# smly/RiichiEnv

Hardware: AMD Instinct MI355X
Metric: env.step()/s (whole node) at 65 536 parallel 4p games; bit-exact MJAI parity (higher is better)
Workload: dtype u8

## Files before the change

riichienv_amd/csrc/rmj_step4.hip.h:

```cpp
namespace RMJ_NS {

#define R4_LIST 16
#define R4_ACT_CAP (KSANMA ? 2 * R4_LIST : R4_LIST)
#define R4_RE_DRAW 1u
#define R4_RE_RESTART 2u
#define R4_RE_PUB 3u
#define R4_RE_YAKU_CLAIMS 4u
#define R4_RE_YAKU_TSUMO 5u
#define R4_RE_WIN_TSUMO 6u
#define R4_RE_WIN_RON 7u
#define R4_RET_ROUND 0x100u
#define STEP_F_ROWS_SHIFT 20
__device__ __forceinline__ uint32_t r4_rows(uint32_t flags) {
    const uint32_t c = (flags >> STEP_F_ROWS_SHIFT) & 3u;
    return c == 0u ? 4u : c;
}
#ifdef RMJ_CUTS
#define R4M(id) do { if (rmj::g_cut == (id)) asm volatile("s_endpgm" ::: "memory"); } while (0)
#define R4BAIL(q, id) do { (q).bail = true; if ((q).r == 0) atomicAdd(&rmj::g_bail_reason[id], 1u); } while (0)
#else
#define R4M(id) do {} while (0)
#ifdef RMJ_CENSUS
#define R4BAIL(q, id) do { (q).bail = true; (q).why = (id); } while (0)
#elif defined(RMJ_TL4)
// ... 939 lines not shown
            need_tp = false;
        }
        if (RICH && __ballot(need_tp)) {
            if (need_tp) {
                tp = r4_tenpai_keep(q, P, full, hl);
                if (r == 0 && !r_stage) { G->tp_seat = (uint8_t)pid; G->tp_mask = (uint16_t)tp; G->tp_step = G->step_count + 1u; }
            }
        }
        const bool ok = r < hl && !forb && (!r_stage || ((tp >> r) & 1u));
        const uint32_t vb = rballot(ok, rb);
        if (ok) r4_put(q, pid, n + __popc(vb & ((1u << r) - 1u)), mk_action(RMJ_DISCARD, ht, 0), r4_tile_id(hty));
        n += __popc(vb);
        if (riichi_pre && tp != 0u) {
            if (r == 0) r4_put(q, pid, n, mk_action(RMJ_RIICHI, RMJ_TILE_NONE, 0), KSANMA ? 27 : 37);
            n += 1;
        }
    }
    R4M(61);
    if (drawable > 0 && drawn) {
        if (!r_decl && !r_stage) {
            const bool any4 = (((full.a | full.b | full.c) & O9_4) | (full.d & O7_4)) != 0u;
            if (any4) {
                const int next_t = __builtin_amdgcn_update_dpp(0xFFFF, ht, 0x101 , 0xf, 0xf, false);
                if (rballot(r < hl - 2 && ht > next_t, rb)) { R4BAIL(q, 15); return; }
                const int prev_ty = __builtin_amdgcn_update_dpp(-1, hty, 0x111 , 0xf, 0xf, false);
                const bool is4 = r < hl - 1 && hty != prev_ty && ph_cnt(full, hty) == 4;
                const uint32_t ab = rballot(is4, rb);
                if (is4) {
                    const uint32_t lo = (uint32_t)hty * 4u;
                    r4_put(q, pid, n + __popc(ab & ((1u << r) - 1u)), mk_action(RMJ_ANKAN, lo, 4, lo, lo + 1, lo + 2, lo + 3),
                           (KSANMA ? 29 : 42) + r4_tile_id(hty));
                }
                n += __popc(ab);
            }
            const uint32_t pon_lane = rballot(r < nmelds && P->meld_type[r & 3] == RMJ_MELD_PON, rb);
            if (pon_lane) {
                for (int m = 0; m < nmelds; m++) {
                    if (P->meld_type[m] != RMJ_MELD_PON) continue;
                    const int target = P->meld_tiles[m][0] >> 2;
                    const bool hit = r < hl && hty == target;
                    const uint32_t kb = rballot(hit, rb);
                    if (hit)
                        r4_put(q, pid, n + __popc(kb & ((1u << r) - 1u)),
                               mk_kakan(ht, P->meld_tiles[m][0], P->meld_tiles[m][1], P->meld_tiles[m][2]),
                               (KSANMA ? 29 : 42) + r4_tile_id(target));
                    n += __popc(kb);
                }
            }
        } else if (r_decl) {
            if (ph_cnt(full, drawn_tile >> 2) == 4) { R4BAIL(q, 16); return; }
        }
    }
    if (G->is_first_turn && !r_stage && (G->p[0].n_melds | G->p[1].n_melds | G->p[2].n_melds | G->p[3].n_melds) == 0) {
        const bool term = r < hl && is_terminal_tile136(ht);
        const uint32_t lo = row_or16(term && hty < 32 ? 1u << hty : 0u), hi = row_or16(term && hty >= 32 ? 1u << (hty - 32) : 0u);
        const int kinds = __popc((uint32_t)rbc((int)lo, rb + 15)) + __popc((uint32_t)rbc((int)hi, rb + 15));
        if (kinds >= 9) {
            if (r == 0) r4_put(q, pid, n, mk_action(RMJ_KYUSHU, RMJ_TILE_NONE, 0), KSANMA ? 57 : 80);
            n += 1;
        }
    }
    if (KSANMA && drawn && drawable > 0) {
        const bool hit = r < hl && hty == 30;
        const uint32_t kb = rballot(hit, rb);
        if (hit) r4_put(q, pid, n + __popc(kb & ((1u << r) - 1u)), mk_action(RMJ_KITA, ht, 0), 59);
        n += __popc(kb);
    }
    if (n > R4_ACT_CAP) { R4BAIL(q, 17); return; }
    nl_mine = r == pid ? n : 0;
    wave_sync();
}

__device__ __forceinline__ void r4_emit_now(R4& q, bool on, uint32_t w) {
    if (q.E->skip_log) return;
    const uint32_t evc = q.G->ev_count;
    wave_sync();
    if (on) {
        uint32_t* dst = reinterpret_cast<uint32_t*>(q.E->events + (size_t)q.g * (q.E->ring_mask + 1u) + (evc & q.E->ring_mask));
        if (q.r < 8) dst[q.r] = q.r == 7 ? ((w & 0x00FFFFFFu) | ((uint32_t)KNP << 24)) : w;
        if (q.r == 0) q.G->ev_count = evc + 1u;
    }
    wave_sync();
}
#ifdef RMJ_RE_PROF
#define RE_MARK(k) do { const unsigned long long t__ = __builtin_amdgcn_s_memrealtime(); if (lane == 0) atomicAdd(&rmj::g_re_prof[k], t__ - re_t); re_t = t__; } while (0)
#define RE_ROWS(md) do { if ((threadIdx.x & 15u) == 0u) atomicAdd(&rmj::g_re_prof[8 + ((md) & 15u)], 1ull); } while (0)
#define RE_STAMP(t) const unsigned long long t = __builtin_amdgcn_s_memrealtime()
#define RE_ROUND_END_DONE(t) do { if ((threadIdx.x & 63u) == 0u) { const unsigned long long tr = __builtin_amdgcn_s_memrealtime(); atomicAdd(&rmj::g_re_prof[0], tr - t); atomicAdd(&rmj::g_re_prof[1], 1ull); atomicAdd(&rmj::g_re_prof[17], t); atomicAdd(&rmj::g_re_prof[19], tr); } } while (0)
#define RE_PASS2_DONE(t) do { if ((threadIdx.x & 63u) == 0u) { atomicAdd(&rmj::g_re_prof[2], __builtin_amdgcn_s_memrealtime() - t); atomicAdd(&rmj::g_re_prof[3], 1ull); } } while (0)
#else
#define RE_MARK(k) do {} while (0)
#define RE_ROWS(md) do {} while (0)
#define RE_STAMP(t) do {} while (0)
#define RE_ROUND_END_DONE(t) do {} while (0)
#define RE_PASS2_DONE(t) do {} while (0)
#endif
template <bool RICH>
__device__ __noinline__ void r4_round_end(const Env* Ep, uint32_t g0) {
    const int lane = threadIdx.x & 63, row = lane >> 4, r = lane & 15, rb = lane & 48;
#ifdef RMJ_RE_PROF
    unsigned long long re_t = __builtin_amdgcn_s_memrealtime();
    if (lane == 0) atomicAdd(&rmj::g_re_prof[16], re_t);
#endif
    Quad4Shared& sh = g_q4;
    const uint32_t mode = sh.rmode[row];
    CEnv& E = *(CEnv*)uni_ptr(Ep);
    g0 = uni(g0);
    GState* G = &sh.st[row];
    R4 q;
    q.G = G; q.T = &sh.u.t; q.E = &E; q.lane = lane; q.r = r; q.rb = rb; q.row = row; q.g = g0 + (uint32_t)row;
    q.live = mode != 0u; q.bail = false; q.cont = 0; q.rend = mode; q.evn = 0; q.dirty = 0xFu; q.pause_ok = false; q.yk = 0u; q.yk_mode = 0u; q.gf = false;
    const bool draw = mode == R4_RE_DRAW, restart = mode == R4_RE_RESTART;
    const bool win_t = mode == R4_RE_WIN_TSUMO, win_r = mode == R4_RE_WIN_RON, win = win_t || win_r;
    bool newround = restart;
    int n_oya = 0, n_rw = 0, n_honba = 0;
    uint32_t n_sticks = 0u;
    const bool seat = r < KNP;
    const int oya = G->oya;
    bool oya_won = false;
    if (RICH && __ballot(win)) {
        const uint8_t* Wg = E.wall + (size_t)q.g * RMJ_WALL_STRIDE;
        const uint32_t rules = E.rule_bits;
        const bool from_discard = G->last_discard_pid != 0xFF;
        const int target = (win_r && from_discard) ? (int)G->last_discard_pid : (int)G->current_player;
        const int win_tile = win_t ? (G->drawn_tile != 0xFF ? (int)G->drawn_tile : 0) : (from_discard ? (int)G->last_discard_tile : 0);
        const uint32_t ron_m = win_r ? (sh.yk[row] & 0xFu) : 0u;
        const uint32_t honba0 = G->honba;
        int32_t total_d = 0;
        bool honba_taken = false, deposit_taken = false;
        for (int dist = 0; dist < KNP; dist++) {
            int w = target + dist;
            w = w >= KNP ? w - KNP : w;
            const bool on = dist == 0 ? win_t : (win_r && ((ron_m >> w) & 1u) != 0u);
            if (!__ballot(on)) continue;
            const PState& Wp = G->p[w & 3];
            const uint32_t wfl = on ? (uint32_t)Wp.flags : 0u;
            const bool riichi = (wfl & PF_RIICHI_DECLARED) != 0u;
            uint32_t cf = (riichi ? CF_RIICHI : 0u) | ((wfl & PF_DOUBLE_RIICHI) ? CF_DOUBLE_RIICHI : 0u) | ((wfl & PF_IPPATSU) ? CF_IPPATSU : 0u);
            const bool last_tile = G->drawable_count == 0 && !G->is_rinshan;
            if (win_t) {
                cf |= CF_TSUMO;
                if (last_tile) cf |= CF_HAITEI;
                if (G->is_rinshan) cf |= CF_RINSHAN;
                const bool no_melds = (G->p[0].n_melds | G->p[1].n_melds | G->p[2].n_melds | G->p[3].n_melds) == 0;
                if (G->is_first_turn && no_melds) cf |= CF_FIRST_TURN;
            } else {
                if (last_tile) cf |= CF_HOUTEI;
                if (G->pending_kan_pid != 0xFF && a_type(G->pending_kan_action) != RMJ_KITA) cf |= CF_CHANKAN;
            }
            const uint32_t hb = honba_taken ? 0u : honba0;
            if (on) honba_taken = true;
            E4Out o = r4_seat_eval<true>(on ? 1u : 0u, (uint32_t)w, (uint32_t)win_tile, cf, hb, riichi, Wg);
            const bool w_oya = w == oya;
            if (o.yakuman && o.han > 13) {
                int cap = 0;
                if (((o.ym >> 47) & 1ull) && !(rules & RMJ_RULE_JUNSEI_CHUUREN_DOUBLE)) cap += 13;
                if (((o.ym >> 48) & 1ull) && !(rules & RMJ_RULE_SUUANKOU_TANKI_DOUBLE)) cap += 13;
                if (((o.ym >> 49) & 1ull) && !(rules & RMJ_RULE_KOKUSHI13_DOUBLE)) cap += 13;
                if (((o.ym >> 50) & 1ull) && !(rules & RMJ_RULE_DAISUUSHII_DOUBLE)) cap += 13;
                if (cap > 0) {
                    const int hh = o.han > cap ? o.han - cap : 0;
                    o.han = hh < 13 ? 13 : hh;
                    const ScoreOut s2 = calc_score((uint32_t)o.han, 0u, w_oya, win_t, hb, (uint32_t)KNP);
                    o.ron = s2.ron; o.tsumo_oya = s2.tsumo_oya; o.tsumo_ko = s2.tsumo_ko;
                }
            }
            const bool won = on && o.is_win;
            int total_val = 0, pao_val = 0, pao_seat = -1;
            if (won && o.yakuman) {
                const uint64_t ids = (0x7FFull << 35) | (0xFull << 47);
                total_val = __popcll(o.ym & ids);
                if (((o.ym >> 47) & 1ull) && (rules & RMJ_RULE_JUNSEI_CHUUREN_DOUBLE)) total_val += 1;
                if (((o.ym >> 48) & 1ull) && (rules & RMJ_RULE_SUUANKOU_TANKI_DOUBLE)) total_val += 1;
                if (((o.ym >> 49) & 1ull) && (rules & RMJ_RULE_KOKUSHI13_DOUBLE)) total_val += 1;
                const int v50 = (rules & RMJ_RULE_DAISUUSHII_DOUBLE) ? 2 : 1;
                if (((o.ym >> 50) & 1ull) && v50 == 2) total_val += 1;
                if (((o.ym >> 37) & 1ull) && Wp.pao37 != 0xFF) { pao_val += 1; pao_seat = Wp.pao37; }
                if (((o.ym >> 50) & 1ull) && Wp.pao50 != 0xFF) { pao_val += v50; pao_seat = Wp.pao50; }
            }
            const int32_t sticks = (won && !deposit_taken) ? (int32_t)(G->riichi_sticks * 1000u) : 0;
            int32_t d = 0;
// ... 311 lines not shown
        }
        wave_sync();
#pragma unroll
        for (int k = 0; k < 3; k++) {
            const int i = lane + 64 * k;
            if (i < N) {
                const uint32_t b = (uint32_t)(key[k] >> 57);
                const uint32_t kw = (((uint32_t)(key[k] >> 49) & 0xFFu) << 8) | (uint32_t)i;
                const int lo = off8[b], hi = b == 127u ? N : (int)off8[b + 1u];
                int rk = lo;
                for (int t = lo; t < hi; t++) {
                    const uint32_t kt = gk[t];
                    bool less = kt < kw;
                    if ((kt >> 8) == (kw >> 8) && kt != kw) {
                        const uint32_t it = kt & 0xFFu;
                        const uint64_t kf = sm64(hs + (uint64_t)it * 0x9E3779B97F4A7C15ull);
                        less = kf < key[k] || (kf == key[k] && it < (uint32_t)i);
                    }
                    rk += less ? 1 : 0;
                }
                place(rk, (KSANMA && i >= 4) ? i + 28 : i);
            }
        }
        if (lane < (RMJ_WALL_STRIDE - N)) Wg[N + lane] = 0;
        }
        wave_sync();
        {
            const int sp = lane >> 4, sl = lane & 15;
            const bool in = sp < KNP && sl < 13;
            const int t = in ? (int)Gb->p[sp & 3].hand[sl] : 0xFFFF;
            int rk = 0;
#pragma unroll
            for (int k = 0; k < 13; k++) rk += rbc(t, rb + k) < t ? 1 : 0;
            wave_sync();
            if (in) Gb->p[sp & 3].hand[rk] = (uint8_t)t;
            if (sp < KNP && sl == 0) Gb->p[sp & 3].hand_len = sp == oya ? 14 : 13;
        }
        if (lane == 0) {
            Gb->hand_index = hidx + 1u;
            Gb->live_end = (uint8_t)(N - 13 * KNP - 1);
            Gb->drawable_count = (uint8_t)(N - 13 * KNP - 14 - 1);
            Gb->needs_tsumo = 0;
            Gb->phase = RMJ_WAIT_ACT;
            Gb->active_mask = (uint8_t)(1u << oya);
        }
        wave_sync();
        if (!E.skip_log) {
            const uint32_t evc = Gb->ev_count, ring = E.ring_mask + 1u;
            RmjEvent* ring0 = E.events + (size_t)gb * ring;
            if (lane < 8) {
                const uint32_t ks = Gb->riichi_sticks;
                uint32_t w = 0u;
                if (lane == 0) w = (uint32_t)RMJ_EV_START_KYOKU | ((uint32_t)oya << 8) | ((uint32_t)(oya + 1) << 16) | ((uint32_t)Gb->dora[0] << 24);
                if (lane == 1) w = ((uint32_t)Gb->round_wind & 3u) | ((uint32_t)Gb->honba << 8) | ((ks & 0xFFu) << 16) | (((ks >> 8) & 0xFFu) << 24);
                if (lane >= 2 && lane < 2 + KNP) w = (uint32_t)Gb->p[(lane - 2) & 3].score;
                if (lane == 7) w = (uint32_t)KNP << 24;
                reinterpret_cast<uint32_t*>(ring0 + (evc & E.ring_mask))[lane] = w;
            }
            {
                const int rec = lane >> 5, b = lane & 31;
                uint32_t v = 0u;
                if (b == 0) v = RMJ_EV_TEHAI;
                if (b == 1) v = (uint32_t)rec;
                if (b >= 4 && b < 30) {
                    const int j = b - 4, sp = 2 * rec + (j >= 13 ? 1 : 0), k = j >= 13 ? j - 13 : j;
                    v = sp < KNP ? Gb->p[sp & 3].hand[k] : 0u;
                }
                if (b == 31) v = (uint32_t)KNP;
                reinterpret_cast<uint8_t*>(ring0 + ((evc + 1u + (uint32_t)rec) & E.ring_mask))[b] = (uint8_t)v;
            }
            if (lane < 8) {
                uint32_t w = 0u;
                if (lane == 0) w = (uint32_t)RMJ_EV_TSUMO | ((uint32_t)oya << 8) | ((uint32_t)Gb->drawn_tile << 24);
                if (lane == 7) w = (uint32_t)KNP << 24;
                reinterpret_cast<uint32_t*>(ring0 + ((evc + 3u) & E.ring_mask))[lane] = w;
            }
            wave_sync();
            if (lane == 0) Gb->ev_count = evc + 4u;
        }
        wave_sync();
    }
#ifdef RMJ_RE_PROF
    if (lane == 0) { const unsigned long long te = __builtin_amdgcn_s_memrealtime(); atomicAdd(&rmj::g_re_prof[5], te - pw0); atomicAdd(&rmj::g_re_prof[18], te); }
#endif
}

__device__ __noinline__ void r4_yaku_answers() {
    const int lane = threadIdx.x & 63, row = lane >> 4, r = lane & 15, rb = lane & 48;
    Quad4Shared& sh = g_q4;
    const GState* G = &sh.st[row];
    const uint32_t mode = sh.rmode[row];
    const bool claims = mode == R4_RE_YAKU_CLAIMS, tsumo = mode == R4_RE_YAKU_TSUMO;
    uint32_t todo = 0u;
    const int tile = claims ? (int)G->last_discard_tile : (int)G->drawn_tile;
    if (__ballot(claims)) {
        const int pid = G->last_discard_pid, tt = tile >> 2;
        const PState& S4 = G->p[r & 3];
        const bool other = claims && r < KNP && r != pid;
        const uint32_t qfl = S4.flags;
        const bool holds13 = other && (S4.hand_len + 3 * S4.n_melds == 13);
        const uint64_t W = holds13 ? S4.waits13 : 0ull;
        const uint64_t dtm = S4.discard_type_mask;
        const bool in_discards = (dtm >> tt) & 1ull;
        const bool in_missed = (qfl & PF_MISSED_DOUJUN) || ((qfl & PF_RIICHI_DECLARED) && (qfl & PF_MISSED_RIICHI));
        const bool furiten = (W & dtm) != 0ull || (qfl & (PF_MISSED_RIICHI | PF_MISSED_DOUJUN));
        const uint32_t riichi_m = rballot(r < 4 && (qfl & PF_RIICHI_DECLARED), rb) & 0xFu;
        todo = rballot(other && !in_discards && !in_missed && !furiten && ((W >> tt) & 1ull), rb) & 0xFu & ~riichi_m;
    }
    if (tsumo) todo = 1u << G->current_player;
    uint32_t ok_m = 0u, miss_m = 0u, han_m = 0u;
    while (__ballot(todo != 0u)) {
        const uint32_t on = todo != 0u ? 1u : 0u;
        const int i = on ? __ffs((int)todo) - 1 : 0;
        todo &= todo - 1u;
        const uint32_t fl_i = G->p[i].flags;
        uint32_t cf = ((fl_i & PF_RIICHI_DECLARED) ? CF_RIICHI : 0u) | ((fl_i & PF_DOUBLE_RIICHI) ? CF_DOUBLE_RIICHI : 0u) | ((fl_i & PF_IPPATSU) ? CF_IPPATSU : 0u);
        if (tsumo) {
            cf |= CF_TSUMO;
            if (G->drawable_count == 0 && !G->is_rinshan) cf |= CF_HAITEI;
            if (G->is_rinshan) cf |= CF_RINSHAN;
            if (G->is_first_turn && G->p[i].n_discards == 0) cf |= CF_FIRST_TURN;
        } else if (G->drawable_count == 0 && !G->is_rinshan) {
            cf |= CF_HOUTEI;
        }
        const uint32_t res = r4_yaku_check(on, (uint32_t)i, (uint32_t)tile, cf);
        if (on) {
            if (res & 1u) ok_m |= 1u << i;
            else if (res & 2u) miss_m |= 1u << i;
            if (res & 4u) han_m |= 1u << i;
        }
    }
    if (r == 0) sh.yk[row] = tsumo ? (((ok_m & han_m) != 0u) ? 1u : 0u) : (ok_m | (miss_m << 4));
    wave_sync();
}

__device__ __forceinline__ uint32_t r4_prio(uint32_t ty, bool call) {
    const uint32_t lo = call ? 0x90205678u : 0x90205CC8u, hi = 0xFFFF1A43u;
    return __builtin_amdgcn_ubfe(ty < 8u ? lo : hi, (ty & 7u) * 4u, 4u);
}
__device__ __forceinline__ uint32_t sh_triple_1m(uint64_t nv, uint64_t other, uint64_t side, int m) {
    const uint32_t n0 = (uint32_t)nv & 0xFFFFFu, n1 = (uint32_t)(nv >> 20) & 0xFFFFFu;
    const uint32_t o0 = (uint32_t)other & 0xFFFFFu, o1 = (uint32_t)(other >> 20) & 0xFFFFFu;
    const uint32_t s0 = ((uint32_t)side & 0xFFFFFu) | 0xFFF00000u, s1 = ((uint32_t)(side >> 20) & 0xFFFFFu) | 0xFFF00000u;
    uint32_t S0[5], S1[5], N0[5], N1[5], O0[5], O1[5];
#pragma unroll
    for (int j = 0; j < 5; j++) {
        const uint32_t off = m >= j ? 4u * (uint32_t)(m - j) : 20u;
        S0[j] = (s0 >> off) & 15u; S1[j] = (s1 >> off) & 15u;
        N0[j] = __builtin_amdgcn_ubfe(n0, 4u * j, 4u); N1[j] = __builtin_amdgcn_ubfe(n1, 4u * j, 4u);
        O0[j] = __builtin_amdgcn_ubfe(o0, 4u * j, 4u); O1[j] = __builtin_amdgcn_ubfe(o1, 4u * j, 4u);
    }
    uint32_t best = 15u;
#pragma unroll
    for (int k1 = 0; k1 < 5; k1++)
#pragma unroll
        for (int k2 = 0; k1 + k2 < 5; k2++) {
            const int j = k1 + k2;
            best = min(best, N0[k1] + O0[k2] + S1[j]);
            best = min(best, N1[k1] + O0[k2] + S0[j]);
            best = min(best, N0[k1] + O1[k2] + S0[j]);
        }
    return best;
}
__device__ __forceinline__ uint32_t row_min16u(uint32_t v) {
    v = min(v, (uint32_t)__builtin_amdgcn_update_dpp(0x7FFFFFFF, (int)v, 0x111, 0xf, 0xf, false));
    v = min(v, (uint32_t)__builtin_amdgcn_update_dpp(0x7FFFFFFF, (int)v, 0x112, 0xf, 0xf, false));
    v = min(v, (uint32_t)__builtin_amdgcn_update_dpp(0x7FFFFFFF, (int)v, 0x114, 0xf, 0xf, false));
    v = min(v, (uint32_t)__builtin_amdgcn_update_dpp(0x7FFFFFFF, (int)v, 0x118, 0xf, 0xf, false));
// ... 661 lines not shown
                                }
                                const int tv = tile >> 2;
                                if (tv >= 31 && tv <= 33) { if (nd == 3) C->pao37 = (uint8_t)ldp; }
                                else if (tv >= 27 && tv <= 30) { if (nw == 4) C->pao50 = (uint8_t)ldp; }
                            }
                            G->current_player = (uint8_t)claimer;
                            G->phase = RMJ_WAIT_ACT;
                            G->active_mask = (uint8_t)(1u << claimer);
                            C->forbidden[0] = (uint8_t)tile;
                            C->n_forbidden = 1;
                            if (ty != RMJ_PON) {
                                const int t34 = tile >> 2;
                                const int x = (int)c0 >> 2, y = (int)c1 >> 2;
                                const int lo = min(x, y), hi = max(x, y);
                                if (lo == t34 + 1 && hi == t34 + 2) {
                                    if (t34 % 9 <= 5) { C->forbidden[1] = (uint8_t)((t34 + 3) * 4); C->n_forbidden = 2; }
                                } else if (t34 >= 2 && hi == t34 - 1 && lo == t34 - 2 && t34 % 9 >= 3) {
                                    C->forbidden[1] = (uint8_t)((t34 - 3) * 4);
                                    C->n_forbidden = 2;
                                }
                            }
                            G->needs_tsumo = 0;
                            G->drawn_tile = 0xFF;
                        }
                        wave_sync();
                    }
                } else {
                    if (G->pending_kan_pid != 0xFF) {
                        R4BAIL(q, 26);
                    } else {
                        if (r == 0) {
                            G->active_mask = 0;
                            G->ron_offer_mask = 0;
                        }
                        if (r < 4) G->stale_n[r] = 0;
                        wave_sync();
                        r4_accept_riichi(q);
                        const uint32_t tc = G->turn_count + 1u;
                        const int np_ = (G->current_player + 1) % KNP;
                        if (r == 0) {
                            G->turn_count = tc;
                            G->current_player = (uint8_t)np_;
                        }
                        wave_sync();
                        r4_deal_next(q, pf);
                        if (!q.bail) {
                            if (r == 0 && tc >= (uint32_t)KNP) G->is_first_turn = 0;
                            wave_sync();
                        }
                    }
                }
            }
        }
        R4M(43);
    }
    R4T(2);
    bool wait_deal = !pass2 && t0 && !q.bail && q.rend != 0u;
    if (q.rend) q.dirty = 0xFu;
    if (pass2 && RICH && __ballot(t0 && q.yk_mode == R4_RE_YAKU_CLAIMS)) {
        if (t0 && q.yk_mode == R4_RE_YAKU_CLAIMS) {
            r4_resolve_discard<RICH, LOOP, true>(q, G->last_discard_pid, G->last_discard_tile, false, pf, nl_mine, w_mine);
            if (q.bail && q.cont == 0) q.cont = 3;
        }
    }
    if (t0 && !wait_deal) {
        if (!q.bail && G->phase == RMJ_WAIT_ACT && !(q.rend && G->is_done)) {
            nl_mine = 0;
            w_mine = 0ull;
            const PState& Pc = G->p[G->current_player & 3];
            if (!(noop && G->nlegal[G->current_player & 3] == 0 && Pc.hand_len + 3 * Pc.n_melds == 14)) r4_gen_act_legal<RICH>(q, nl_mine);
            if (q.rend && q.bail) q.cont = 2;
        }
        if (!pass2 && !q.bail && q.rend != 0u) wait_deal = true;
    }
    R4M(45);
    R4T(3);
    const bool done0 = q.live && t0 && !q.bail && !wait_deal;
    const uint32_t used = (!q.live || pass2) ? 0u : ((INLR && second && (!q.bail || q.cont)) ? 2u : 1u);
    const uint32_t fl_pub = pass2 ? sh.rfl[row] : (INLR ? (flags | ((final_chunk && left == used) ? STEP_F_ALLROWS : STEP_F_QUIET)) : flags);
    if (r == 0) {
        sh.rmode[row] = wait_deal ? q.rend : 0u;
        sh.rfl[row] = fl_pub;
    }
    if (done0) {
        const uint32_t am = G->active_mask;
        const bool acts = r < 4 && ((am >> r) & 1u);
        const int n_me = acts ? nl_mine : 0;
        const bool quiet = LOOP && (fl_pub & STEP_F_QUIET) != 0u;
        const uint32_t rows = quiet ? 0u : ((LOOP && (fl_pub & STEP_F_ALLROWS)) ? 0xFu : ((rballot(r < 4 && G->nlegal[r & 3] != 0, rb) | am) & 0xFu));
        if (!quiet) q.T->mk[row][r >> 2][r & 3] = 0u;
        wave_sync();
        for (uint32_t m = am; m; m &= m - 1u) {
            const int p = __ffs((int)m) - 1;
            const int n = rbc(n_me, rb + p);
            if (r < n) {
                const uint64_t e = q.T->lst[row][p][r];
                (E.legal + (size_t)g * 4 * RMJ_MAX_LEGAL)[p * RMJ_MAX_LEGAL + r] = e & 0x00FFFFFFFFFFFFFFull;
                const int id = (int)(e >> 56);
                if (!quiet) atomicOr(&q.T->mk[row][p][id >> 5], 1u << (id & 31));
            }
            if (R4_ACT_CAP > R4_LIST && r + R4_LIST < n) {
                const uint64_t e = (&q.T->lst[row][p][0])[r + R4_LIST];
                (E.legal + (size_t)g * 4 * RMJ_MAX_LEGAL)[p * RMJ_MAX_LEGAL + r + R4_LIST] = e & 0x00FFFFFFFFFFFFFFull;
                const int id = (int)(e >> 56);
                if (!quiet) atomicOr(&q.T->mk[row][p][id >> 5], 1u << (id & 31));
            }
        }
        wave_sync();
        uint16_t* mout = reinterpret_cast<uint16_t*>(E.mask + (size_t)g * 328);
        for (uint32_t m = rows; m; m &= m - 1u) {
            const int p = __ffs((int)m) - 1;
#pragma unroll
            for (int k = 0; k < 3; k++) {
                const int j = r + 16 * k;
                if (j < 41) {
                    const uint32_t w = q.T->mk[row][p][(2 * j) >> 5];
                    const uint32_t b0 = (w >> ((2 * j) & 31)) & 1u, b1 = (w >> ((2 * j + 1) & 31)) & 1u;
                    mout[41 * p + j] = (uint16_t)(b0 | (b1 << 8));
                }
            }
        }
        if (r < 4) {
            if (!quiet) E.nlegal[(size_t)g * 4 + r] = (uint8_t)n_me;
            G->nlegal[r] = (uint8_t)n_me;
            if (!quiet) E.waits[(size_t)g * 4 + r] = acts ? w_mine : 0ull;
            if (acts && !G->is_done) {
                G->obs_from[r] = G->obs_upto[r];
                G->obs_upto[r] = G->ev_count;
            }
        }
        if (r == 0 && !quiet) E.status[g] = (uint32_t)G->active_mask | ((uint32_t)G->phase << 8) | ((uint32_t)G->is_done << 16);
        if (r < 2 * q.evn) {
            const int e = r >> 1, hh = r & 1;
            uint4* dst = reinterpret_cast<uint4*>(E.events + (size_t)g * (E.ring_mask + 1u) + q.T->evidx[row][e]);
            dst[hh] = reinterpret_cast<const uint4*>(q.T->ev[row][e])[hh];
        }
    }
    if (q.live && (q.cont || wait_deal) && r < 2 * q.evn) {
        const int e = r >> 1, hh = r & 1;
        uint4* dst = reinterpret_cast<uint4*>(E.events + (size_t)g * (E.ring_mask + 1u) + q.T->evidx[row][e]);
        dst[hh] = reinterpret_cast<const uint4*>(q.T->ev[row][e])[hh];
    }
    wave_sync();
    R4M(46);
    R4T(4);
    if (done0) {
#pragma unroll
        for (int k = 0; k < 3; k++) {
            const int off = r + 16 * k;
            if (off < (int)(sizeof(GState) / 16) && (off >= 32 || ((q.dirty >> (off >> 3)) & 1u)))
                reinterpret_cast<uint4*>(E.core + g)[off] = reinterpret_cast<const uint4*>(&sh.st[row])[off];
        }
    }
    wave_sync();
    R4M(47);
    R4T(5);
    uint64_t bm = __ballot(q.live && q.bail && r == 0);
    const uint32_t fl_full = ((INLR || pass2) ? fl_pub : flags) |
                             (q.cont == 1 ? STEP_F_CONT_RYU : 0u) | (q.cont == 2 ? STEP_F_CONT_FIN : 0u) | (q.cont == 3 ? STEP_F_CONT_CLAIMS : 0u);
#ifdef RMJ_TL4
    if (!LOOP && lane == 0) rmj::g_tl4[(size_t)blockIdx.x * RMJ_TL4_ROW + 7] = (unsigned long long)__popcll(bm);
#endif
    while (bm) {
        const int br = (__ffsll((long long)bm) - 1) >> 4;
        bm &= bm - 1ull;
        const uint32_t gg = g0 + (uint32_t)br;
#ifdef RMJ_CENSUS
        {
            const int why_b = __builtin_amdgcn_readlane(q.cont == 2 ? 31 : q.why, 16 * br);
            if (lane == 0) atomicAdd(&rmj::g_bail_reason[why_b & 31], 1u);
        }
#endif
        const uint64_t m_full = rbc64(mine, 16 * br + (lane & 3));
        Ctx c{sh.st[br], E, sh.u.x, gg, lane, E.wall + (size_t)gg * RMJ_WALL_STRIDE, E.legal + (size_t)gg * 4 * RMJ_MAX_LEGAL};
#ifdef RMJ_TL4
        if (lane < 16) sh.u.x.tl_acc[lane] = 0u;
        if (lane == 0) sh.u.x.tl_prev = __builtin_readcyclecounter();
        wave_sync();
#endif
        if (LOOP) __builtin_amdgcn_fence(__ATOMIC_ACQUIRE, "agent");
        ol_step_full(ctx_pack(c), lane < 4 ? m_full : RMJ_NO_ACTION, (uint32_t)__builtin_amdgcn_readlane((int)fl_full, 16 * br));
        wave_sync();
#ifdef RMJ_TL4
        if (!LOOP && lane < 16) rmj::g_tl4[(size_t)blockIdx.x * RMJ_TL4_ROW + 16 + lane] += (unsigned long long)sh.u.x.tl_acc[lane];
        wave_sync();
#endif
    }
    R4T(6);
    if (LOOP) {
        __builtin_amdgcn_fence(__ATOMIC_RELEASE, "workgroup");
        wave_sync();
    }
    return used | (__ballot(wait_deal) ? R4_RET_ROUND : 0u);
    }
}
template <bool LOOP, int POL>
__device__ __noinline__ void step4_pass2(const Env* Ep, uint32_t flags, uint32_t g_base, uint32_t g_end, uint32_t quad = 0xFFFFFFFFu) {
    Quad4Shared& sh = g_q4;
    step4_body<LOOP, POL, false, true>(uni_ptr(Ep), sh, 0ull, uni(flags), uni(g_base), uni(g_end), false, 0ull, nullptr, uni(quad));
}
template <bool LOOP, int POL>
__device__ __forceinline__ void step4_finish_rounds(const Env* Ep, uint32_t flags, uint32_t g_base, uint32_t g_end, uint32_t quad = 0xFFFFFFFFu) {
    constexpr bool RICH = (POL == 1) || !LOOP;
    const uint32_t md = g_q4.rmode[(threadIdx.x & 63u) >> 4];
    RE_ROWS(md);
    if (__ballot(md == R4_RE_DRAW || md == R4_RE_RESTART || md == R4_RE_WIN_TSUMO || md == R4_RE_WIN_RON)) {
        if (LOOP && RICH) __builtin_amdgcn_fence(__ATOMIC_ACQUIRE, "agent");
        RE_STAMP(pt0);
        r4_round_end<RICH>(Ep, g_base + (quad == 0xFFFFFFFFu ? blockIdx.x : quad) * r4_rows(flags));
        RE_ROUND_END_DONE(pt0);
    }
    if (RICH && __ballot(md == R4_RE_YAKU_CLAIMS || md == R4_RE_YAKU_TSUMO)) r4_yaku_answers();
    RE_STAMP(pt1);
    step4_pass2<LOOP, POL>(Ep, flags, g_base, g_end, quad);
    RE_PASS2_DONE(pt1);
}
template <int POL>
__device__ __forceinline__ uint32_t step4_call_inl(const Env* Ep, uint64_t policy_seed, uint32_t flags, uint32_t g_base, uint32_t g_end, uint32_t load,
                                                   uint64_t gs_row, uint32_t quad, uint32_t left, uint32_t final_chunk) {
    Quad4Shared& sh = g_q4;
    Ep = uni_ptr(Ep); policy_seed = uni(policy_seed); flags = uni(flags); g_base = uni(g_base); g_end = uni(g_end); quad = uni(quad); final_chunk = uni(final_chunk);
    asm volatile("" : "+s"(Ep), "+s"(policy_seed), "+s"(flags), "+s"(g_base), "+s"(g_end), "+s"(quad), "+s"(final_chunk));
    return step4_body<true, POL, true>(uni_ptr(Ep), sh, uni(policy_seed), uni(flags), uni(g_base), uni(g_end), uni(load) != 0u, gs_row, nullptr, uni(quad),
                                       left, uni(final_chunk) != 0u);
}
template <int POL>
__device__ __forceinline__ uint32_t step4_run(const Env* Ep, uint64_t policy_seed, uint32_t flags, uint32_t g_base, uint32_t g_end, uint64_t gs_row,
                                              uint32_t quad, uint32_t steps, bool final_chunk, uint32_t g_row, uint32_t max_calls = 0xFFFFFFFFu) {
    uint32_t left = g_row < g_end ? steps : 0u, load = 1u;
#ifdef RMJ_QTL
    if ((threadIdx.x & 63u) == 0u) { g_qtl_cnt[0] = 0u; g_qtl_cnt[1] = 0u; }
#endif
#pragma unroll 1
    while (__ballot(left != 0u) && max_calls-- != 0u) {
#ifdef RMJ_QTL
        { const uint64_t lv = __ballot(left != 0u && (threadIdx.x & 15u) == 0u); if ((threadIdx.x & 63u) == 0u) { g_qtl_cnt[0] += 1u; g_qtl_cnt[1] += (uint32_t)__popcll(lv); } }
#endif
        const uint32_t ret = step4_call_inl<POL>(Ep, policy_seed, flags, g_base, g_end, load, gs_row, quad, left, final_chunk ? 1u : 0u);
        left -= ret & 0xFFu;
        load = 0u;
        if (__ballot((ret & R4_RET_ROUND) != 0u)) step4_finish_rounds<true, POL>(Ep, flags, g_base, g_end, quad);
    }
    return left;
}
#define RMJ_STEP4_WAVES 6
#define RMJ_STEP4_WAVES_GREEDY 5
#define RMJ_STEP4_WAVES_OF(POL) ((POL) == 1 ? RMJ_STEP4_WAVES_GREEDY : RMJ_STEP4_WAVES)
template <bool LOOP, int POL>
__global__ __launch_bounds__(64, (LOOP && POL == 1) ? RMJ_STEP4_WAVES_GREEDY : RMJ_STEP4_WAVES) void k_step4(const Env* __restrict__ Ep, uint64_t policy_seed, uint32_t flags, uint32_t g_base,
                                                                   uint32_t g_end, uint32_t n_steps, const uint64_t* __restrict__ actions, HeavyOrder ho) {
    if (LOOP) {
        const uint32_t row_ = (threadIdx.x & 63u) >> 4;
        const uint32_t g = row_ < r4_rows(flags) ? g_base + blockIdx.x * r4_rows(flags) + row_ : 0xFFFFFFFFu;
        const uint64_t gs_row = sm64(policy_seed + ((CEnv*)Ep)->game_offset + (uint64_t)g);
        step4_run<POL>(Ep, policy_seed, flags, g_base, g_end, gs_row, 0xFFFFFFFFu, n_steps, true, g);
    } else {
        Quad4Shared& sh = g_q4;
#ifdef RMJ_TL4
        const unsigned long long rt0 = __builtin_amdgcn_s_memrealtime();
#endif
        uint32_t unit = blockIdx.x;
        if (ho.in_cnt) {
            if (blockIdx.x == 0 && (threadIdx.x & 63) == 0) *ho.zero_cnt = 0u;
            if (blockIdx.x < ho.front) {
                if (blockIdx.x >= uni(*ho.in_cnt)) return;
                unit = uni(ho.in_list[blockIdx.x]);
            } else {
                unit = blockIdx.x - ho.front;
                if (uni((uint32_t)ho.in_flag[unit])) return;
            }
        }
        const uint32_t ret = step4_body<false, POL>(Ep, sh, policy_seed, flags, g_base, g_end, true, 0ull, actions, unit);
#ifdef RMJ_TL4
        if ((threadIdx.x & 63) == 0) rmj::g_tl4[(size_t)blockIdx.x * RMJ_TL4_ROW + 15] = __ballot((ret & R4_RET_ROUND) != 0u) ? 1ull : 0ull;
        if (__ballot((ret & R4_RET_ROUND) != 0u) && (threadIdx.x & 63) == 0)
            rmj::g_tl4[(size_t)blockIdx.x * RMJ_TL4_ROW + 14] = (1ull << g_q4.rmode[0]) | (1ull << g_q4.rmode[1]) | (1ull << g_q4.rmode[2]) | (1ull << g_q4.rmode[3]);
#endif
        if (__ballot((ret & R4_RET_ROUND) != 0u)) step4_finish_rounds<false, POL>(Ep, flags, g_base, g_end, unit);
        if (ho.out_cnt) {
            const int row = (threadIdx.x & 63) >> 4;
            const GState& S = sh.st[row];
            const uint32_t gq = g_base + unit * r4_rows(flags) + (uint32_t)row;
            const PState& Pw = S.p[threadIdx.x & 3];
            const bool waits_open = (threadIdx.x & 15) < 4 && (Pw.flags & PF_WAITS_VALID) && Pw.waits13 != 0ull && !(Pw.flags & PF_RIICHI_DECLARED);
            const bool hv = (uint32_t)row < r4_rows(flags) && gq < g_end &&
                            (S.is_done ? (flags & STEP_F_AUTORESET) != 0u : ((S.phase == RMJ_WAIT_ACT && S.drawable_count == 0) || S.ron_offer_mask != 0 || waits_open));
            const bool any = __ballot(hv) != 0ull;
            if ((threadIdx.x & 63) == 0) {
                uint32_t idx = 0xFFFFFFFFu;
                if (any) idx = atomicAdd(ho.out_cnt, 1u);
                if (idx < ho.front) ho.out_list[idx] = unit;
                ho.out_flag[unit] = idx < ho.front ? 1 : 0;
            }
        }
#ifdef RMJ_TL4
        const unsigned long long rt1 = __builtin_amdgcn_s_memrealtime();
        if ((threadIdx.x & 63) == 0) {
            rmj::g_tl4[(size_t)blockIdx.x * RMJ_TL4_ROW + 8] = rt0;
            rmj::g_tl4[(size_t)blockIdx.x * RMJ_TL4_ROW + 9] = rt1;
        }
#endif
    }
}

#define RMJ_Q_STRIDE 32u
__device__ __noinline__ uint32_t q_take_ticket(uint32_t* head) {
    uint32_t t = 0u;
    if ((threadIdx.x & 63u) == 0u) t = __hip_atomic_fetch_add(head, 1u, __ATOMIC_RELAXED, __HIP_MEMORY_SCOPE_AGENT);
    return (uint32_t)__builtin_amdgcn_readfirstlane((int)t);
}
#define RMJ_Q_FIN 0x80000000u
__device__ __noinline__ uint32_t q_wait_for(const uint32_t* slot, uint32_t want) {
    uint32_t v = 0u;
    if ((threadIdx.x & 63u) == 0u)
        for (;;) {
            v = __hip_atomic_load(slot, __ATOMIC_RELAXED, __HIP_MEMORY_SCOPE_AGENT);
            if ((v & RMJ_Q_FIN) || v >= want) break;
            __builtin_amdgcn_s_sleep(8);
        }
    wave_sync();
    return (uint32_t)__builtin_amdgcn_readfirstlane((int)v);
}
template <int POL>
__global__ __launch_bounds__(64, RMJ_STEP4_WAVES_OF(POL)) void k_step4_queue(const Env* __restrict__ Ep, uint64_t policy_seed, uint32_t flags, uint32_t n_games,
// ... 178 lines not shown
```

Before: 2.087 billion.

## Serve round-end legal generation and publish inline, skipping pass2 for lean tier

```diff
diff --git a/riichienv_amd/csrc/rmj_step4.hip.h b/riichienv_amd/csrc/rmj_step4.hip.h
--- a/riichienv_amd/csrc/rmj_step4.hip.h
+++ b/riichienv_amd/csrc/rmj_step4.hip.h
@@ -1045,6 +1045,92 @@
     }
     wave_sync();
 }
+#ifdef RMJ_TL4
+#define R4T_PARAM , uint64_t& tl_prev
+#define R4T_ARG , tl_prev
+#else
+#define R4T_PARAM
+#define R4T_ARG
+#endif
+template <bool LOOP>
+__device__ __forceinline__ void r4_publish(R4& q, Quad4Shared& sh, const bool done0, const bool wait_deal, const uint32_t fl_pub, const int nl_mine,
+                                           const uint64_t w_mine R4T_PARAM) {
+    CEnv& E = *q.E;
+    GState* G = q.G;
+    const int r = q.r, rb = q.rb, row = q.row;
+    const uint32_t g = q.g;
+    if (done0) {
+        const uint32_t am = G->active_mask;
+        const bool acts = r < 4 && ((am >> r) & 1u);
+        const int n_me = acts ? nl_mine : 0;
+        const bool quiet = LOOP && (fl_pub & STEP_F_QUIET) != 0u;
+        const uint32_t rows = quiet ? 0u : ((LOOP && (fl_pub & STEP_F_ALLROWS)) ? 0xFu : ((rballot(r < 4 && G->nlegal[r & 3] != 0, rb) | am) & 0xFu));
+        if (!quiet) q.T->mk[row][r >> 2][r & 3] = 0u;
+        wave_sync();
+        for (uint32_t m = am; m; m &= m - 1u) {
+            const int p = __ffs((int)m) - 1;
+            const int n = rbc(n_me, rb + p);
+            if (r < n) {
+                const uint64_t e = q.T->lst[row][p][r];
+                (E.legal + (size_t)g * 4 * RMJ_MAX_LEGAL)[p * RMJ_MAX_LEGAL + r] = e & 0x00FFFFFFFFFFFFFFull;
+                const int id = (int)(e >> 56);
+                if (!quiet) atomicOr(&q.T->mk[row][p][id >> 5], 1u << (id & 31));
+            }
+            if (R4_ACT_CAP > R4_LIST && r + R4_LIST < n) {
+                const uint64_t e = (&q.T->lst[row][p][0])[r + R4_LIST];
+                (E.legal + (size_t)g * 4 * RMJ_MAX_LEGAL)[p * RMJ_MAX_LEGAL + r + R4_LIST] = e & 0x00FFFFFFFFFFFFFFull;
+                const int id = (int)(e >> 56);
+                if (!quiet) atomicOr(&q.T->mk[row][p][id >> 5], 1u << (id & 31));
+            }
+        }
+        wave_sync();
+        uint16_t* mout = reinterpret_cast<uint16_t*>(E.mask + (size_t)g * 328);
+        for (uint32_t m = rows; m; m &= m - 1u) {
+            const int p = __ffs((int)m) - 1;
+#pragma unroll
+            for (int k = 0; k < 3; k++) {
+                const int j = r + 16 * k;
+                if (j < 41) {
+                    const uint32_t w = q.T->mk[row][p][(2 * j) >> 5];
+                    const uint32_t b0 = (w >> ((2 * j) & 31)) & 1u, b1 = (w >> ((2 * j + 1) & 31)) & 1u;
+                    mout[41 * p + j] = (uint16_t)(b0 | (b1 << 8));
+                }
+            }
+        }
+        if (r < 4) {
+            if (!quiet) E.nlegal[(size_t)g * 4 + r] = (uint8_t)n_me;
+            G->nlegal[r] = (uint8_t)n_me;
+            if (!quiet) E.waits[(size_t)g * 4 + r] = acts ? w_mine : 0ull;
+            if (acts && !G->is_done) {
+                G->obs_from[r] = G->obs_upto[r];
+                G->obs_upto[r] = G->ev_count;
+            }
+        }
+        if (r == 0 && !quiet) E.status[g] = (uint32_t)G->active_mask | ((uint32_t)G->phase << 8) | ((uint32_t)G->is_done << 16);
+        if (r < 2 * q.evn) {
+            const int e = r >> 1, hh = r & 1;
+            uint4* dst = reinterpret_cast<uint4*>(E.events + (size_t)g * (E.ring_mask + 1u) + q.T->evidx[row][e]);
+            dst[hh] = reinterpret_cast<const uint4*>(q.T->ev[row][e])[hh];
+        }
+    }
+    if (q.live && (q.cont || wait_deal) && r < 2 * q.evn) {
+        const int e = r >> 1, hh = r & 1;
+        uint4* dst = reinterpret_cast<uint4*>(E.events + (size_t)g * (E.ring_mask + 1u) + q.T->evidx[row][e]);
+        dst[hh] = reinterpret_cast<const uint4*>(q.T->ev[row][e])[hh];
+    }
+    wave_sync();
+    R4M(46);
+    R4T(4);
+    if (done0) {
+#pragma unroll
+        for (int k = 0; k < 3; k++) {
+            const int off = r + 16 * k;
+            if (off < (int)(sizeof(GState) / 16) && (off >= 32 || ((q.dirty >> (off >> 3)) & 1u)))
+                reinterpret_cast<uint4*>(E.core + g)[off] = reinterpret_cast<const uint4*>(&sh.st[row])[off];
+        }
+    }
+    wave_sync();
+}
 #ifdef RMJ_RE_PROF
 #define RE_MARK(k) do { const unsigned long long t__ = __builtin_amdgcn_s_memrealtime(); if (lane == 0) atomicAdd(&rmj::g_re_prof[k], t__ - re_t); re_t = t__; } while (0)
 #define RE_ROWS(md) do { if ((threadIdx.x & 15u) == 0u) atomicAdd(&rmj::g_re_prof[8 + ((md) & 15u)], 1ull); } while (0)
@@ -1058,8 +1144,8 @@
 #define RE_ROUND_END_DONE(t) do {} while (0)
 #define RE_PASS2_DONE(t) do {} while (0)
 #endif
-template <bool RICH>
-__device__ __noinline__ void r4_round_end(const Env* Ep, uint32_t g0) {
+template <bool RICH, bool SERVE>
+__device__ __forceinline__ void r4_round_end_impl(const Env* Ep, uint32_t g0) {
     const int lane = threadIdx.x & 63, row = lane >> 4, r = lane & 15, rb = lane & 48;
 #ifdef RMJ_RE_PROF
     unsigned long long re_t = __builtin_amdgcn_s_memrealtime();
@@ -1537,8 +1623,26 @@
     }
 #ifdef RMJ_RE_PROF
     if (lane == 0) { const unsigned long long te = __builtin_amdgcn_s_memrealtime(); atomicAdd(&rmj::g_re_prof[5], te - pw0); atomicAdd(&rmj::g_re_prof[18], te); }
+    re_t = __builtin_amdgcn_s_memrealtime();
 #endif
-}
+    if constexpr (SERVE) {
+        int nl_mine = 0;
+        q.gf = true;
+        if (newround) r4_gen_act_legal<false>(q, nl_mine);
+        const bool done0 = newround && !q.bail;
+#ifdef RMJ_TL4
+        uint64_t tl_prev = __builtin_readcyclecounter();
+#endif
+        r4_publish<true>(q, sh, done0, false, sh.rfl[row], nl_mine, 0ull R4T_ARG);
+        if (done0 && r == 0) sh.rmode[row] = 0u;
+        __builtin_amdgcn_fence(__ATOMIC_RELEASE, "workgroup");
+        wave_sync();
+        RE_MARK(7);
+    }
+}
+template <bool RICH>
+__device__ __noinline__ void r4_round_end(const Env* Ep, uint32_t g0) { r4_round_end_impl<RICH, false>(Ep, g0); }
+__device__ __noinline__ void r4_round_serve(const Env* Ep, uint32_t g0) { r4_round_end_impl<false, true>(Ep, g0); }
 
 __device__ __noinline__ void r4_yaku_answers() {
     const int lane = threadIdx.x & 63, row = lane >> 4, r = lane & 15, rb = lane & 48;
@@ -2366,77 +2470,7 @@
         sh.rmode[row] = wait_deal ? q.rend : 0u;
         sh.rfl[row] = fl_pub;
     }
-    if (done0) {
-        const uint32_t am = G->active_mask;
-        const bool acts = r < 4 && ((am >> r) & 1u);
-        const int n_me = acts ? nl_mine : 0;
-        const bool quiet = LOOP && (fl_pub & STEP_F_QUIET) != 0u;
-        const uint32_t rows = quiet ? 0u : ((LOOP && (fl_pub & STEP_F_ALLROWS)) ? 0xFu : ((rballot(r < 4 && G->nlegal[r & 3] != 0, rb) | am) & 0xFu));
-        if (!quiet) q.T->mk[row][r >> 2][r & 3] = 0u;
-        wave_sync();
-        for (uint32_t m = am; m; m &= m - 1u) {
-            const int p = __ffs((int)m) - 1;
-            const int n = rbc(n_me, rb + p);
-            if (r < n) {
-                const uint64_t e = q.T->lst[row][p][r];
-                (E.legal + (size_t)g * 4 * RMJ_MAX_LEGAL)[p * RMJ_MAX_LEGAL + r] = e & 0x00FFFFFFFFFFFFFFull;
-                const int id = (int)(e >> 56);
-                if (!quiet) atomicOr(&q.T->mk[row][p][id >> 5], 1u << (id & 31));
-            }
-            if (R4_ACT_CAP > R4_LIST && r + R4_LIST < n) {
-                const uint64_t e = (&q.T->lst[row][p][0])[r + R4_LIST];
-                (E.legal + (size_t)g * 4 * RMJ_MAX_LEGAL)[p * RMJ_MAX_LEGAL + r + R4_LIST] = e & 0x00FFFFFFFFFFFFFFull;
-                const int id = (int)(e >> 56);
-                if (!quiet) atomicOr(&q.T->mk[row][p][id >> 5], 1u << (id & 31));
-            }
-        }
-        wave_sync();
-        uint16_t* mout = reinterpret_cast<uint16_t*>(E.mask + (size_t)g * 328);
-        for (uint32_t m = rows; m; m &= m - 1u) {
-            const int p = __ffs((int)m) - 1;
-#pragma unroll
-            for (int k = 0; k < 3; k++) {
-                const int j = r + 16 * k;
-                if (j < 41) {
-                    const uint32_t w = q.T->mk[row][p][(2 * j) >> 5];
-                    const uint32_t b0 = (w >> ((2 * j) & 31)) & 1u, b1 = (w >> ((2 * j + 1) & 31)) & 1u;
-                    mout[41 * p + j] = (uint16_t)(b0 | (b1 << 8));
-                }
-            }
-        }
-        if (r < 4) {
-            if (!quiet) E.nlegal[(size_t)g * 4 + r] = (uint8_t)n_me;
-            G->nlegal[r] = (uint8_t)n_me;
-            if (!quiet) E.waits[(size_t)g * 4 + r] = acts ? w_mine : 0ull;
-            if (acts && !G->is_done) {
-                G->obs_from[r] = G->obs_upto[r];
-                G->obs_upto[r] = G->ev_count;
-            }
-        }
-        if (r == 0 && !quiet) E.status[g] = (uint32_t)G->active_mask | ((uint32_t)G->phase << 8) | ((uint32_t)G->is_done << 16);
-        if (r < 2 * q.evn) {
-            const int e = r >> 1, hh = r & 1;
-            uint4* dst = reinterpret_cast<uint4*>(E.events + (size_t)g * (E.ring_mask + 1u) + q.T->evidx[row][e]);
-            dst[hh] = reinterpret_cast<const uint4*>(q.T->ev[row][e])[hh];
-        }
-    }
-    if (q.live && (q.cont || wait_deal) && r < 2 * q.evn) {
-        const int e = r >> 1, hh = r & 1;
-        uint4* dst = reinterpret_cast<uint4*>(E.events + (size_t)g * (E.ring_mask + 1u) + q.T->evidx[row][e]);
-        dst[hh] = reinterpret_cast<const uint4*>(q.T->ev[row][e])[hh];
-    }
-    wave_sync();
-    R4M(46);
-    R4T(4);
-    if (done0) {
-#pragma unroll
-        for (int k = 0; k < 3; k++) {
-            const int off = r + 16 * k;
-            if (off < (int)(sizeof(GState) / 16) && (off >= 32 || ((q.dirty >> (off >> 3)) & 1u)))
-                reinterpret_cast<uint4*>(E.core + g)[off] = reinterpret_cast<const uint4*>(&sh.st[row])[off];
-        }
-    }
-    wave_sync();
+    r4_publish<LOOP>(q, sh, done0, wait_deal, fl_pub, nl_mine, w_mine R4T_ARG);
     R4M(47);
     R4T(5);
     uint64_t bm = __ballot(q.live && q.bail && r == 0);
@@ -2483,18 +2517,21 @@
     Quad4Shared& sh = g_q4;
     step4_body<LOOP, POL, false, true>(uni_ptr(Ep), sh, 0ull, uni(flags), uni(g_base), uni(g_end), false, 0ull, nullptr, uni(quad));
 }
-template <bool LOOP, int POL>
+template <bool LOOP, int POL, bool SERVE = false>
 __device__ __forceinline__ void step4_finish_rounds(const Env* Ep, uint32_t flags, uint32_t g_base, uint32_t g_end, uint32_t quad = 0xFFFFFFFFu) {
     constexpr bool RICH = (POL == 1) || !LOOP;
+    static_assert(!SERVE || !RICH, "the round service is the lean tier's");
     const uint32_t md = g_q4.rmode[(threadIdx.x & 63u) >> 4];
     RE_ROWS(md);
     if (__ballot(md == R4_RE_DRAW || md == R4_RE_RESTART || md == R4_RE_WIN_TSUMO || md == R4_RE_WIN_RON)) {
         if (LOOP && RICH) __builtin_amdgcn_fence(__ATOMIC_ACQUIRE, "agent");
         RE_STAMP(pt0);
-        r4_round_end<RICH>(Ep, g_base + (quad == 0xFFFFFFFFu ? blockIdx.x : quad) * r4_rows(flags));
+        if constexpr (SERVE) r4_round_serve(Ep, g_base + (quad == 0xFFFFFFFFu ? blockIdx.x : quad) * r4_rows(flags));
+        else r4_round_end<RICH>(Ep, g_base + (quad == 0xFFFFFFFFu ? blockIdx.x : quad) * r4_rows(flags));
         RE_ROUND_END_DONE(pt0);
     }
     if (RICH && __ballot(md == R4_RE_YAKU_CLAIMS || md == R4_RE_YAKU_TSUMO)) r4_yaku_answers();
+    if (SERVE && !__ballot(g_q4.rmode[(threadIdx.x & 63u) >> 4] != 0u)) return;
     RE_STAMP(pt1);
     step4_pass2<LOOP, POL>(Ep, flags, g_base, g_end, quad);
     RE_PASS2_DONE(pt1);
@@ -2523,7 +2560,7 @@
         const uint32_t ret = step4_call_inl<POL>(Ep, policy_seed, flags, g_base, g_end, load, gs_row, quad, left, final_chunk ? 1u : 0u);
         left -= ret & 0xFFu;
         load = 0u;
-        if (__ballot((ret & R4_RET_ROUND) != 0u)) step4_finish_rounds<true, POL>(Ep, flags, g_base, g_end, quad);
+        if (__ballot((ret & R4_RET_ROUND) != 0u)) step4_finish_rounds<true, POL, POL == 0>(Ep, flags, g_base, g_end, quad);
     }
     return left;
 }
```

Result: no change. 2.112 billion (median of 6 runs) (+1.2%).
